# Lingeng56/conformer-pytorch-lightning

Measured on AMD Instinct MI355X. Metric: encoder frames/sec (80-d fbank, T=1000), whole job, higher is better.
Workload: dtype bf16

## Files before the change

conformer-pytorch-lightning_amd/cfm/__init__.py:

```python
import ctypes
import os
import threading

import torch

_HERE = os.path.dirname(os.path.abspath(__file__))
LIB_PATH = os.path.join(os.path.dirname(_HERE), "libconformer_gfx950.so")

F32, BF16, F16 = 0, 1, 2
ACT_NONE, ACT_SILU, ACT_RELU, ACT_GLU, ACT_DSILU, ACT_DRELU = 0, 1, 2, 3, 4, 5
TILE_AUTO_TRAIN = -1

_DT = {torch.float32: F32, torch.bfloat16: BF16, torch.float16: F16}
_TORCH_DT = {F32: torch.float32, BF16: torch.bfloat16, F16: torch.float16}

c_p = ctypes.c_void_p
c_i64 = ctypes.c_int64
c_i32 = ctypes.c_int32
c_f = ctypes.c_float


class GemmDesc(ctypes.Structure):
    _fields_ = [("A", c_p), ("W", c_p), ("W_lo", c_p), ("bias", c_p), ("residual", c_p), ("row_mask", c_p), ("C", c_p),
                ("lda", c_i64), ("ldc", c_i64), ("ldr", c_i64),
# ... 244 lines not shown
        L.cfm_dwconv_bn_train_bwd_acc.argtypes = [c_p, c_i32, c_p, c_p, c_p, c_i32, c_p, c_p, c_i32, c_p, c_p, c_p, c_p, c_p, c_p, c_i32, c_i32, c_i32, c_i32, c_i32, c_p]
        L.cfm_layernorm_bwd_fused.argtypes = [ctypes.POINTER(LnBwdDesc), c_p]
        L.cfm_conv12_relu.argtypes = [c_p, c_p, c_p, c_p, c_p, c_p, c_i32, c_i32, c_i32, c_i32, c_i32, c_p, c_p, c_p]
        L.cfm_valid_mask.argtypes = [c_p, c_i32, c_p, c_i32, c_i32, c_i32, c_i32, c_p]
        L.cfm_chunk_mask.argtypes = [c_p, c_i32, c_i32, c_i32, c_p]
        L.cfm_attn_mask.argtypes = [c_p, c_p, c_p, c_i32, c_i32, c_p]
        L.cfm_cast.argtypes = [c_p, c_i32, c_p, c_i32, c_i64, c_p]
        L.cfm_add_rows.argtypes = [c_p, c_p, c_i64, c_i32, c_i32, c_p]
        L.cfm_encoder_layer_forward.argtypes = [ctypes.POINTER(LayerWeights), ctypes.POINTER(LayerScratch),
                                                ctypes.POINTER(LayerIO), c_p, c_p, c_i32, c_p, c_p, c_p]
        L.cfm_encoder_layer_route.argtypes = [ctypes.POINTER(LayerWeights), ctypes.POINTER(LayerScratch), ctypes.POINTER(LayerIO), c_p, c_p]
        L.cfm_encoder_layer_route.restype = c_i32
        L.cfm_ffsplit_max_rows.restype = c_i32
        L.cfm_ctc_nll.argtypes = [c_p, c_i64, c_i32, c_i32, c_i32, c_p, c_p, c_i32, c_p, c_p, c_p, c_p]
        L.cfm_joint_act.argtypes = [c_p, c_i64, c_p, c_i64, c_p, c_i32, c_i32, c_i32, c_i32, c_i32, c_p]
        L.cfm_joint_act_bwd.argtypes = [c_p, c_i64, c_p, c_i64, c_p, c_p, c_p, c_p, c_i32, c_i32, c_i32, c_i32, c_p]
        L.cfm_joint_act_bwd_ws.argtypes = [c_i32, c_i32, c_i32, c_i32]
        L.cfm_rnnt_nll.argtypes = [ctypes.POINTER(RnntDesc), c_p]
        L.cfm_rnnt_grad.argtypes = [ctypes.POINTER(RnntDesc), c_p]
        L.cfm_rnnt_packed_nll.argtypes = [ctypes.POINTER(RnntPackedDesc), c_p]
        L.cfm_rnnt_packed_grad.argtypes = [ctypes.POINTER(RnntPackedDesc), c_p]
        L.cfm_joint_act_packed.argtypes = [c_p, c_i64, c_p, c_i64, c_p, c_i32, ctypes.POINTER(Lattice), c_i32, c_p]
        L.cfm_joint_act_packed_bwd.argtypes = [c_p, c_i64, c_p, c_i64, c_p, c_p, c_p, c_p, ctypes.POINTER(Lattice), c_i32, c_p]
        c_f = ctypes.c_float
        L.cfm_gemm_tn.argtypes = [ctypes.POINTER(GemmTnDesc), c_p]
        L.cfm_gemm_tn_group.argtypes = [ctypes.POINTER(GemmTnDesc), c_i32, c_p]
        L.cfm_attention_bwd.argtypes = [ctypes.POINTER(AttnBwdDesc), c_p]
        L.cfm_layernorm_bwd_ws.argtypes = [c_i64, c_i32]
        L.cfm_layernorm_bwd.argtypes = [c_p, c_p, c_i32, c_p, c_p, c_p, c_p, c_p, c_p, c_p, c_f, c_i64, c_i32, c_p]
        L.cfm_glu_bwd.argtypes = [c_p, c_i32, c_p, c_i32, c_p, c_i32, c_i64, c_i32, c_p]
        L.cfm_dwconv_bn_ws.argtypes = [c_i32, c_i32, c_i32]
        L.cfm_dwconv_bn_train.argtypes = [c_p, c_i32, c_p, c_p, c_p, c_p, c_p, c_p, c_f, c_f, c_p, c_p, c_p, c_i32, c_p, c_i32, c_i32, c_i32, c_i32, c_p]
        L.cfm_dwconv_bn_train_bwd.argtypes = [c_p, c_i32, c_p, c_p, c_p, c_i32, c_p, c_p, c_i32, c_p, c_p, c_p, c_p, c_p, c_p, c_i32, c_i32, c_i32, c_i32, c_p]
        L.cfm_col2im_relu_bwd.argtypes = [c_p, c_i32, c_p, c_i32, c_p, c_i32, c_i32, c_i32, c_i32, c_i32, c_p]
        L.cfm_conv1_wgrad_ws.argtypes = [c_i32, c_i32, c_i32]
        L.cfm_conv1_wgrad.argtypes = [c_p, c_i32, c_p, c_p, c_p, c_p, c_p, c_p, c_i32, c_i32, c_i32, c_i32, c_p]
        L.cfm_ctc_nll_train_groups.argtypes = [ctypes.POINTER(CtcGroup), c_i32, c_i32, c_p]
        L.cfm_ctc_grad.argtypes = [c_p, c_i64, c_i32, c_i32, c_i32, c_p, c_p, c_i32, c_p, c_p, c_p, c_p, c_p, c_p, c_f, c_p, c_p, c_p]
        L.cfm_adam_step.argtypes = [c_p, c_p, c_p, c_p, c_i64, c_f, c_f, c_f, c_f, c_f, c_i64, c_p, c_p]
        L.cfm_sumsq.argtypes = [c_p, c_i64, c_p, c_i32, c_p, c_p]
        L.cfm_adam_clip_step.argtypes = [c_p, c_p, c_p, c_p, c_i64, c_f, c_f, c_f, c_f, c_f, c_i64, c_p, c_f, c_f, c_i32, c_p, c_p]
        L.cfm_dropout_rows.argtypes = [c_p, c_i32, c_p, c_i32, c_p, c_f, c_f, ctypes.c_uint32, c_f, ctypes.c_uint32, c_i64, c_i32, c_p]
        L.cfm_dropout_mask.argtypes = [c_p, c_i64, c_f, ctypes.c_uint32, c_p]
        L.cfm_encoder_train_forward.argtypes = [c_i32, ctypes.POINTER(LayerTrainWeights), ctypes.POINTER(LayerTrainIO), ctypes.POINTER(LayerTrainSaved),
                                                ctypes.POINTER(LayerTrainScratch), ctypes.POINTER(c_p), c_p]
        L.cfm_encoder_train_backward.argtypes = [c_i32, ctypes.POINTER(LayerTrainWeights), ctypes.POINTER(LayerTrainIO), ctypes.POINTER(LayerTrainSaved),
                                                 ctypes.POINTER(LayerTrainScratch), ctypes.POINTER(LayerTrainGrads), ctypes.POINTER(c_p), c_p, c_p, c_p,
                                                 LAYER_DONE_FN, c_p, ctypes.POINTER(c_p), c_p]
        L.cfm_stream_prep.argtypes = [c_p, c_i32, c_i32, c_i32, c_i32, c_p, c_i32, c_i32, c_p, c_p, c_p, c_p]
        L.cfm_kv_ring_write.argtypes = [c_p, c_p, c_i32, c_i64, c_i64, c_i64, c_i64, c_p, c_p, c_i32, c_i32, c_i32, c_i32, c_i32, c_p]
        L.cfm_stream_advance.argtypes = [c_p, c_p, c_i32, c_i32, c_p]
        L.cfm_dwconv_causal_bn_silu.argtypes = [c_p, c_i32, c_p, c_p, c_p, c_p, c_p, c_p, c_i32, c_i32, c_i32, c_i32, c_i32, c_p]
        L.cfm_conv_cache_update.argtypes = [c_p, c_i32, c_p, c_i32, c_i32, c_i32, c_i32, c_p]
        for name in ("cfm_layernorm_bwd_ws", "cfm_dwconv_bn_ws", "cfm_conv1_wgrad_ws", "cfm_joint_act_bwd_ws"):
            getattr(L, name).restype = c_i64
        L.cfm_prof_enable.argtypes = [c_i32]
        L.cfm_prof_enable.restype = None
        L.cfm_prof_reset.restype = None
        L.cfm_prof_collect.restype = ctypes.c_int
        L.cfm_prof_entry.argtypes = [c_i32, ctypes.c_char_p, c_i32, ctypes.POINTER(c_i64), ctypes.POINTER(ctypes.c_double),
                                     ctypes.POINTER(ctypes.c_double), ctypes.POINTER(ctypes.c_double)]
        for name in ("cfm_gemm", "cfm_ffn_fused", "cfm_rowchain", "cfm_rowchain_supported", "cfm_attention", "cfm_layernorm", "cfm_kv_cache_pack", "cfm_dwconv_bn_silu", "cfm_conv1_relu", "cfm_conv1_relu_mma", "cfm_conv12_relu", "cfm_conv12_supported",
                     "cfm_valid_mask", "cfm_chunk_mask", "cfm_attn_mask", "cfm_cast", "cfm_add_rows",
                     "cfm_encoder_layer_forward", "cfm_ctc_nll", "cfm_joint_act", "cfm_joint_act_bwd", "cfm_rnnt_nll", "cfm_rnnt_grad", "cfm_prof_entry", "cfm_gemm_tn", "cfm_gemm_tn_group", "cfm_attention_bwd",
                     "cfm_layernorm_bwd", "cfm_glu_bwd", "cfm_dwconv_bn_train", "cfm_dwconv_bn_train_bwd", "cfm_col2im_relu_bwd", "cfm_conv1_wgrad",
                     "cfm_ctc_nll_train_groups", "cfm_ctc_grad", "cfm_adam_step", "cfm_adam_clip_step", "cfm_sumsq", "cfm_dropout_rows", "cfm_dropout_mask", "cfm_pack_matrices", "cfm_pack_vectors", "cfm_greedy_step", "cfm_greedy_chunk_begin", "cfm_greedy_chunk_step", "cfm_fbank", "cfm_fbank_stream", "cfm_ffn_split", "cfm_ffn_split_supported", "cfm_layernorm_bwd_fused", "cfm_dwconv_bn_train_bwd_acc",
                     "cfm_encoder_train_forward", "cfm_encoder_train_backward", "cfm_stream_prep", "cfm_kv_ring_write", "cfm_stream_advance", "cfm_dwconv_causal_bn_silu", "cfm_conv_cache_update"):
            getattr(L, name).restype = ctypes.c_int
        _lib = L
    return _lib


def check(rc, what):
    if rc != 0:
        raise RuntimeError("%s failed (status %d): %s" % (what, rc, lib().cfm_last_error().decode(errors="replace")))


def dt_code(t):
    try:
        return _DT[t.dtype if isinstance(t, torch.Tensor) else t]
    except KeyError:
        raise TypeError("cfm: unsupported dtype %s (float32, bfloat16, float16 only)" % (t.dtype if isinstance(t, torch.Tensor) else t))


def torch_dtype(code):
    return _TORCH_DT[code]


def require_hip(*tensors):
    for t in tensors:
        if t is None:
            continue
        if not t.is_cuda:
            raise RuntimeError("cfm: tensor on %s -- this framework runs on MI355X (HIP) only; there is no CPU path" % t.device)


def ptr(t):
    return None if t is None else t.data_ptr()


def stream():
    return torch.cuda.current_stream().cuda_stream


class Precision:

# ... 50 lines not shown
```

conformer-pytorch-lightning_amd/cfm/ops.py:

```python
import ctypes

import torch

import cfm as _c

__all__ = ["fbank", "fbank_stream", "stream_prep", "stream_advance", "dwconv_causal_bn_silu", "conv_cache_update", "dropout_rows", "dropout_mask", "set_deterministic", "gemm_tn", "gemm_tn_group", "layernorm_bwd", "glu_bwd", "dwconv_bn_train", "dwconv_bn_train_bwd", "col2im_relu_bwd", "conv1_wgrad", "attention_bwd",
           "ctc_nll_train_groups", "ctc_grad", "rnnt_nll", "rnnt_grad", "joint_act_bwd", "rnnt_nll_packed", "joint_act_packed", "joint_act_packed_bwd", "ffn_split", "adam_step", "adam_clip_step", "sumsq", "scratch_stats",
           "gemm", "ffn_fused", "ffn_fused_supported", "rowchain", "rowchain_supported", "rowchain_pair_supported", "layernorm", "attention", "kv_cache_pack", "dwconv_bn_silu", "conv1_relu", "conv1_relu_mma_supported", "conv12_relu", "conv12_supported", "ctc_nll", "joint_act", "valid_mask", "chunk_mask",
           "attn_mask_combine", "cast", "add_rows", "scratch", "prof_enable", "prof_reset", "prof_table", "as_u8_mask"]


def _rows2d(t, name):
    if t.dim() != 2 or t.stride(1) != 1:
        raise ValueError("cfm.%s: expected a 2-D tensor with unit inner stride, got shape %s strides %s" % (name, tuple(t.shape), t.stride()))
    return t


def _dense(name, **tensors):
    for k, t in tensors.items():
        if t is not None and not t.is_contiguous():
            raise ValueError("cfm.%s: %s must be contiguous (the C ABI has no stride for it), got shape %s strides %s" % (name, k, tuple(t.shape), t.stride()))


def _strides_match(name, what, t, sb, st):
    if t is None:
        return
    if t.dim() not in (2, 3):
        bad = t.stride(-1) != 1
    else:
        bad = t.stride(-1) != 1 or (t.size(-2) > 1 and t.stride(-2) != st) or (t.dim() == 3 and t.size(0) > 1 and t.stride(0) != sb)
    if bad:
        raise ValueError("cfm.%s: %s has strides %s but the call passes (batch %d, time %d) with unit inner stride" % (name, what, t.stride(), sb, st))


_arena = {}
_retired = []


def scratch(tag, numel, dtype, device):
    device = torch.device(device)
    key = (tag, dtype, device, torch.cuda.current_stream(device).cuda_stream)
    buf = _arena.get(key)
    if buf is None or buf.numel() < numel:
        want = max(int(numel), 1) if buf is None else max(int(numel), buf.numel() * 3 // 2)
        if buf is not None:
            _retired.append(buf)
        buf = torch.empty(want, dtype=dtype, device=device)
        _arena[key] = buf
    return buf[:numel]


def scratch_stats():
    held = sum(b.numel() * b.element_size() for b in list(_arena.values()) + _retired)
    return len(_arena), len(_retired), held


def gemm(a, w, bias=None, w_lo=None, out=None, out_dtype=None, act=_c.ACT_NONE, residual=None, alpha=1.0, row_mask=None,
         mask_mode=0, conv=None, tile=0, n_out=None, pre_out=None, aux=None, drop=None, drop2=None):
    _c.require_hip(a, w, bias, w_lo, out, residual, row_mask)
    w = _rows2d(w, "gemm(w)")
    N, K = w.shape
    if w.stride(0) != K:
        raise ValueError("cfm.gemm: w must be dense [N,K] (cfm_gemm_desc carries no row stride for W), got shape %s strides %s" % (tuple(w.shape), w.stride()))
    d = _c.GemmDesc()
    if conv is None:
        a = _rows2d(a, "gemm(a)")
        M = a.shape[0]
        if a.shape[1] != K:
            raise ValueError("cfm.gemm: a is %s but w is %s" % (tuple(a.shape), tuple(w.shape)))
        d.lda = a.stride(0)
    else:
        C, T1, F1, T2, F2, M = conv
        if not a.is_contiguous():
            raise ValueError("cfm.gemm(conv): image must be contiguous channels-last [B,T1,F1,C]")
        d.conv_C, d.conv_T1, d.conv_F1, d.conv_T2, d.conv_F2 = C, T1, F1, T2, F2
        d.lda = 0
    cols = N // 2 if act == _c.ACT_GLU else N
    if out is None:
        odt = out_dtype if out_dtype is not None else (residual.dtype if residual is not None else torch.float32)
        out = torch.empty((M, cols), dtype=odt, device=a.device)
    else:
        out = _rows2d(out, "gemm(out)")
        if out.shape[0] != M or out.shape[1] != cols:
            raise ValueError("cfm.gemm: out is %s, expected (%d,%d)" % (tuple(out.shape), M, cols))
    if residual is not None:
        residual = _rows2d(residual, "gemm(residual)")
        if residual.dtype != torch.float32 or out.dtype != torch.float32 or tuple(residual.shape) != (M, cols):
            raise ValueError("cfm.gemm: residual accumulate needs f32 residual/out of shape (%d,%d)" % (M, cols))
        d.ldr = residual.stride(0)
    if bias is not None and (bias.dtype != torch.float32 or bias.numel() != N or not bias.is_contiguous()):
        raise ValueError("cfm.gemm: bias must be contiguous f32 [N]")
    if row_mask is not None and (row_mask.dtype != torch.uint8 or row_mask.numel() != M or not row_mask.is_contiguous()):
        raise ValueError("cfm.gemm: row_mask must be contiguous uint8 [M]")
    if w_lo is not None and (w_lo.shape != w.shape or w_lo.dtype != w.dtype or not w_lo.is_contiguous()):
        raise ValueError("cfm.gemm: w_lo must match w")
    if pre_out is not None:
        _c.require_hip(pre_out)
        pre_out = _rows2d(pre_out, "gemm(pre_out)")
        if tuple(pre_out.shape) != (M, N):
            raise ValueError("cfm.gemm: pre_out is %s, expected (%d,%d)" % (tuple(pre_out.shape), M, N))
        d.C_pre, d.ld_pre, d.pre_dtype = _c.ptr(pre_out), pre_out.stride(0), _c.dt_code(pre_out)
    if aux is not None:
        _c.require_hip(aux)
        aux = _rows2d(aux, "gemm(aux)")
        if tuple(aux.shape) != (M, N):
            raise ValueError("cfm.gemm: aux is %s, expected (%d,%d)" % (tuple(aux.shape), M, N))
        d.aux, d.ld_aux, d.aux_dtype = _c.ptr(aux), aux.stride(0), _c.dt_code(aux)
    if drop is not None and drop[0] > 0.0:
        d.drop_p, d.drop_seed = float(drop[0]), int(drop[1]) & 0xFFFFFFFF
        if drop2 is not None and drop2[0] > 0.0:
            d.drop2_p, d.drop2_seed = float(drop2[0]), int(drop2[1]) & 0xFFFFFFFF
    d.A, d.W, d.W_lo, d.bias, d.residual, d.row_mask, d.C = _c.ptr(a), _c.ptr(w), _c.ptr(w_lo), _c.ptr(bias), _c.ptr(residual), _c.ptr(row_mask), _c.ptr(out)
    d.ldc = out.stride(0)
    d.M, d.N, d.K = M, N, K
    d.a_dtype, d.w_dtype, d.c_dtype = _c.dt_code(a), _c.dt_code(w), _c.dt_code(out)
    d.act, d.alpha, d.tile, d.mask_mode = act, alpha, tile, mask_mode
    _c.check(_c.lib().cfm_gemm(ctypes.byref(d), _c.stream()), "cfm_gemm")
    return out


def ffn_fused_supported(D, FF, prec):
    return (not prec.split) and D in (144, 256) and FF % 32 == 0 and FF <= 2048


def ffn_fused(x, w1f, w2f, b1, b2, FF, act=_c.ACT_SILU, ln=None, alpha=1.0, add_x=False, ln1=None, ln2=None, out_f32=None,
              want_f32=True, out16_dtype=None, eps=1e-5):
    _c.require_hip(x, w1f, w2f, b1, b2, out_f32)
    x = _rows2d(x, "ffn_fused(x)")
    if x.dtype != torch.float32 or not x.is_contiguous():
        raise ValueError("cfm.ffn_fused: x must be contiguous float32 [M,D]")
    M, D = x.shape
    _dense("ffn_fused", w1f=w1f, w2f=w2f, b1=b1, b2=b2, out_f32=out_f32, **{n + "_" + s: t for n, pr in (("ln", ln), ("ln1", ln1), ("ln2", ln2)) if pr is not None
                                                                            for s, t in zip("gb", pr)})
    if out_f32 is not None and (out_f32.dtype != torch.float32 or tuple(out_f32.shape) != (M, D)):
        raise ValueError("cfm.ffn_fused: out_f32 must be float32 (%d,%d)" % (M, D))
    d = _c.FfnDesc()
    d.x, d.w1f, d.w2f, d.b1, d.b2 = _c.ptr(x), _c.ptr(w1f), _c.ptr(w2f), _c.ptr(b1), _c.ptr(b2)
    for name, pair in (("ln", ln), ("ln1", ln1), ("ln2", ln2)):
        if pair is not None:
            setattr(d, name + "_g", _c.ptr(pair[0]))
            setattr(d, name + "_b", _c.ptr(pair[1]))
    if want_f32 and out_f32 is None:
        out_f32 = torch.empty((M, D), dtype=torch.float32, device=x.device)
    out16 = torch.empty((M, D), dtype=out16_dtype, device=x.device) if out16_dtype is not None else None
    d.out_f32, d.out16 = _c.ptr(out_f32), _c.ptr(out16)
    d.M, d.D, d.FF = M, D, FF
    d.w_dtype = _c.dt_code(w1f)
    d.out16_dtype = _c.dt_code(out16) if out16 is not None else 0
    d.act, d.add_x, d.alpha, d.eps = act, 1 if add_x else 0, alpha, eps
    _c.check(_c.lib().cfm_ffn_fused(ctypes.byref(d), _c.stream()), "cfm_ffn_fused")
    return out_f32, out16


def rowchain_supported(D, FF, prec):
    return (not prec.split) and bool(_c.lib().cfm_rowchain_supported(D, FF))


def rowchain_pair_supported(D, FF, prec):
    return (not prec.split) and bool(_c.lib().cfm_rowchain_pair_supported(D, FF))


def ffn_split(x, w_code, mode, psum=None, psum_b2=None, psum_alpha=1.0, ln1=None, ln2=None, rows_out=None, rows2_out=None, ln=None, w1=None, b1=None,
              n1=0, act=_c.ACT_NONE, w2=None, psum_out=None, out16=None, eps=1e-5, ring=None):
    _c.require_hip(x, psum, psum_b2, rows_out, rows2_out, w1, b1, w2, psum_out, out16)
    x = _rows2d(x, "ffn_split(x)")
    M, D = x.shape
    if x.dtype != torch.float32 or not x.is_contiguous():
        raise ValueError("cfm.ffn_split: x must be contiguous float32 rows")
    _dense("ffn_split", psum_b2=psum_b2, rows_out=rows_out, rows2_out=rows2_out, w1=w1, b1=b1, w2=w2, psum_out=psum_out,
           ring_kv=ring[0] if ring is not None else None, ring_offsets=ring[1] if ring is not None else None, **{n + "_" + sfx: t for n, pr in (("ln", ln), ("ln1", ln1), ("ln2", ln2)) if pr is not None for sfx, t in zip("gb", pr)})
# ... 848 lines not shown
```

conformer-pytorch-lightning_amd/cfm/packing.py:

```python
import torch

import cfm as _c


_EPOCH = [0]


def bump_epoch():
    _EPOCH[0] += 1


def _key(tensors, prec):
    return (prec.name, _EPOCH[0]) + tuple((t.data_ptr(), t._version, str(t.device), t.dtype) for t in tensors if t is not None)


class Packed:

    def __init__(self, **kw):
        self.__dict__.update(kw)


class PackCache:
    def __init__(self):
        self._key = None
        self._val = None

    def __reduce__(self):
        return (PackCache, ())

    def get(self, tensors, prec, build):
        k = _key(tensors, prec)
        if k != self._key:
            with torch.no_grad():
                self._val = build()
            self._key = k
        return self._val


MODULE_CACHES = ("_fused", "_grad_layout", "_stack_w", "_stack_g", "_pack_stack_train")


def state_without_caches(state):
    out = {k: v for k, v in state.items() if k not in MODULE_CACHES}
    if "_fused" in state:
        out["_fused"] = None
    return out


def f32(t):
    return t.detach().to(torch.float32).contiguous()


def matrix(w, prec):
    w32 = w.detach().to(torch.float32)
    if prec.split:
        hi = w32.to(torch.bfloat16)
        lo = (w32 - hi.to(torch.float32)).to(torch.bfloat16)
        return hi.contiguous(), lo.contiguous()
    return w32.to(prec.w_dtype).contiguous(), None


def conv_module_vectors(mod):
    D = mod.pointwise_conv2.weight.shape[0]
    dev = mod.pointwise_conv2.weight.device
    opt = lambda t, n, fill: t.detach() if t is not None else torch.full((n,), fill, device=dev)
    return opt(mod.pointwise_conv1.bias, 2 * D, 0.0), opt(mod.depthwise_conv.bias, D, 0.0), opt(mod.norm.weight, D, 1.0), opt(mod.norm.bias, D, 0.0)


def glu_interleave_index(D, device):
    idx = torch.arange(2 * D, device=device)
    return ((idx % 32) // 16) * D + (idx // 32) * 16 + (idx % 16)


def pack_ffn_fragments(w1, w2, dtype):
    FF, D = w1.shape
    ks1 = (D + 31) // 32
    w1p = torch.zeros((FF, ks1 * 32), dtype=torch.float32, device=w1.device)
    w1p[:, :D] = w1.detach().float()
    w1f = w1p.view(FF // 16, 16, ks1, 4, 8).permute(0, 2, 3, 1, 4).contiguous().to(dtype)
    w2f = w2.detach().float().view(D // 16, 16, FF // 32, 2, 4, 4).permute(2, 0, 4, 1, 3, 5).contiguous().to(dtype)
    return w1f.view(-1), w2f.view(-1)


def pack_frag_major(w, dtype):
    N, K = w.shape
    ks = (K + 31) // 32
    wp = torch.zeros((N, ks * 32), dtype=torch.float32, device=w.device)
    wp[:, :K] = w.detach().float()
    return wp.view(N // 16, 16, ks, 4, 8).permute(0, 2, 3, 1, 4).contiguous().to(dtype).view(-1)
# ... 397 lines not shown
```

conformer-pytorch-lightning_amd/csrc/encoder.cpp:

```cpp
#include <math.h>

#include <stdlib.h>

#include "cfm_common.h"

namespace {

const float kEps = 1e-5f;

inline const void* eoff(const void* p, int64_t elems, int dt) { return (const char*)p + elems * cfm_elt_size(dt); }

struct Ctx {
    const cfm_layer_weights* w; const cfm_layer_scratch* s; const cfm_layer_io* io; const float* x_in; float* x_out; cfm_stream_t st;
    int M, D, FF, H, dk, adt, w_dt, Tc, Tk, P;
    bool split, has_pos, ring;
};

int& cin_merge_flag() {
    static int flag = getenv("CFM_CIN_MERGE") == nullptr || atoi(getenv("CFM_CIN_MERGE")) != 0;
    return flag;
}

int ffsplit_max_rows() {
    static const int rows = getenv("CFM_FFSPLIT_MAX_ROWS") ? atoi(getenv("CFM_FFSPLIT_MAX_ROWS")) : CFM_FFSPLIT_MAX_ROWS;
    return rows;
}

bool taps15(const Ctx& c) { return c.io->ktaps == 15 && !c.io->causal_conv; }

#define CFM_TRY(expr) do { int rc__ = (expr); if (rc__ != CFM_OK) return rc__; } while (0)

int select_route(Ctx& c) {
    const cfm_layer_weights* w = c.w; const cfm_layer_scratch* s = c.s; const cfm_layer_io* io = c.io;
    CFM_CHECK_ARG(w && s && io && c.x_in && c.x_out, "cfm_encoder_layer_forward: null pointer");
    CFM_CHECK_ARG(io->B > 0 && io->T > 0 && io->D > 0 && io->H > 0 && io->D % io->H == 0 && io->FF > 0,
                  "cfm_encoder_layer_forward: bad dims B=%d T=%d D=%d H=%d FF=%d", io->B, io->T, io->D, io->H, io->FF);
    CFM_CHECK_ARG(io->D % 16 == 0, "cfm_encoder_layer_forward: D must be a multiple of 16 (GLU interleave)");
    CFM_CHECK_ARG(c.x_in != c.x_out, "cfm_encoder_layer_forward: x_in and x_out must differ (inputs are not mutated)");
    c.M = io->B * io->T; c.D = io->D; c.FF = io->FF; c.H = io->H; c.dk = c.D / c.H; c.adt = io->act_dtype; c.w_dt = io->w_dtype;
    c.split = io->act_dtype == CFM_F32;
    c.has_pos = io->pos_rows > 0 && w->pos_w;
    c.ring = io->kv_ring != nullptr;
    CFM_CHECK_ARG(!c.ring || (io->stream_offset && io->ring_T >= io->T && !io->attn_cache && !io->new_cache),
                  "encoder layer: the K/V ring needs stream_offset and ring_T >= T, and excludes attn_cache / new_cache");
    c.Tc = io->attn_cache ? io->cache_T : 0;
    c.Tk = c.ring ? io->ring_T : c.Tc + io->T;
    c.P = 0;
    if (c.has_pos) {
        CFM_CHECK_ARG((io->pos_embed || io->pos_proj) && (io->pos_shared || io->pos_rows % io->B == 0),
                      "encoder layer: pos_embed rows (%d) must be a multiple of B (%d)", io->pos_rows, io->B);
        c.P = io->pos_shared ? io->pos_rows : io->pos_rows / io->B;
        CFM_CHECK_ARG(!io->pos_shared || c.P == c.Tk, "encoder layer: shared positions need one row per key (%d rows, Tk=%d)", io->pos_rows, c.Tk);
        CFM_CHECK_ARG(c.P == 1 || c.P == c.Tk, "encoder layer: pos_embed gives %d rows per item, need 1 or Tk=%d (attention.py:78-88)", c.P, c.Tk);
    }
    CFM_CHECK_ARG(c.Tc == 0 || io->new_cache, "encoder layer: a KV cache input needs new_cache storage");
// ... 247 lines not shown
    return cfm_rowchain(&fi, c.st);
}

int run_ffsplit(const Ctx& c) {
    const cfm_layer_weights* w = c.w; const cfm_layer_io* io = c.io;
    const bool ring_written = c.ring && c.dk % 4 == 0;
    CFM_TRY(split_ffn(c, true, c.x_in));
    cfm_ffn_split_desc q = split_reduce(c, 1, c.x_in, w->ffm_b2);
    q.ln_g = w->ln_mha_g; q.ln_b = w->ln_mha_b; q.w1 = w->qkv_wf; q.b1 = w->qkv_b; q.N1 = 3 * c.D; q.act = CFM_ACT_NONE; q.out16 = c.s->qkv; q.ldo = 3 * c.D;
    if (ring_written) { q.kv_ring = io->kv_ring; q.ring_offsets = io->stream_offset; q.ring_T = io->ring_T; q.ring_H = c.H; q.ring_Tq = io->T; }
    CFM_TRY(cfm_ffn_split(&q, c.st));
    CFM_TRY(attention(c, ring_written));
    CFM_TRY(conv_in_chain(c));
    CFM_TRY(conv_out(c, taps15(c) && cfm_rowchain_dw_supported(c.D), c.x_out, 0));
    CFM_TRY(split_ffn(c, false, c.x_out));
    cfm_ffn_split_desc r = split_reduce(c, 0, c.x_out, w->ff_b2);
    r.ln1_g = w->ln_final_g; r.ln1_b = w->ln_final_b;
    if (io->after_out) { r.ln2_g = io->after_g; r.ln2_b = io->after_b; r.rows2_out = io->after_out; }
    return cfm_ffn_split(&r, c.st);
}

int run_pair(const Ctx& c) {
    const cfm_layer_weights* w = c.w; const cfm_layer_scratch* s = c.s;
    float* const park = s->psum + (int64_t)2 * c.M * c.D;
    cfm_rowchain_desc m = ffn_chain(c, true, c.x_in);
    m.psum_out = s->psum;
    CFM_TRY(cfm_rowchain(&m, c.st));
    cfm_rowchain_desc q = chain(c, 1.0f);
    q.x = c.x_in; q.psum_in = s->psum; q.psum_b2 = w->ffm_b2; q.psum_alpha = 0.5f; q.out_f32 = c.x_out; q.ln_g = w->ln_mha_g; q.ln_b = w->ln_mha_b; q.tail_pair = 1;
    qkv_tail(q, c, w);
    CFM_TRY(cfm_rowchain(&q, c.st));
    CFM_TRY(attention(c));
    CFM_TRY(conv_in_chain(c, park));
    CFM_TRY(conv_out(c, taps15(c), park, 1));
    cfm_rowchain_desc fa = ffn_chain(c, false, c.x_out);
    fa.psum_out = s->psum;
    CFM_TRY(cfm_rowchain(&fa, c.st));
    cfm_rowchain_desc fr = chain(c, 1.0f);
    fr.x = c.x_out; fr.psum_in = s->psum; fr.psum_b2 = w->ff_b2; fr.psum_alpha = 0.5f; fr.ln_g = w->ln_final_g; fr.ln_b = w->ln_final_b; fr.out2_f32 = c.x_out;
    CFM_TRY(cfm_rowchain(&fr, c.st));
    return after_norm(c);
}

}

extern "C" int32_t cfm_set_cin_merge(int32_t on) {
    const int prev = cin_merge_flag();
    cin_merge_flag() = on != 0;
    return prev;
}

extern "C" int32_t cfm_ffsplit_max_rows(void) { return ffsplit_max_rows(); }

extern "C" int32_t cfm_encoder_layer_route(const cfm_layer_weights* w, const cfm_layer_scratch* s, const cfm_layer_io* io, const float* x_in, const float* x_out) {
    Ctx c = {w, s, io, x_in, const_cast<float*>(x_out), nullptr};
    return select_route(c);
}

extern "C" int cfm_encoder_layer_forward(const cfm_layer_weights* w, const cfm_layer_scratch* s, const cfm_layer_io* io,
                                         const float* x_in, float* x_out, int xn_ready, const float* next_g,
                                         const float* next_b, cfm_stream_t stream) {
    Ctx c = {w, s, io, x_in, x_out, stream};
    const int route = select_route(c);
    switch (route) {
        case CFM_ROUTE_GENERAL: return run_general(c, xn_ready, next_g, next_b);
        case CFM_ROUTE_FUSED_FFN: return run_fused_ffn(c);
        case CFM_ROUTE_CHAIN: return run_chain(c);
        case CFM_ROUTE_CHAIN_NEXT: return run_chain_next(c);
        case CFM_ROUTE_CHAIN_NEXT_CIN: return run_chain_next_cin(c);
        case CFM_ROUTE_FFSPLIT: return run_ffsplit(c);
        case CFM_ROUTE_PAIR: return run_pair(c);
        default: return route;
    }
}
```

conformer-pytorch-lightning_amd/encoder.py:

```python
import torch
import torch.nn as nn

import cfm
from attention import PositionalEncoding, RelativePositionalEncoding
from convolution import ConvolutionSubSampling
from encoder_layer import ConformerEncoderLayer
from utils import make_attn_mask, make_pad_mask

_NO_MASK = torch.ones((0, 0, 0))


class ConformerEncoder(nn.Module):

    def __init__(self, input_dim, kernel_size, encoder_dim, dropout, attention_dropout, pos_enc_dropout, hidden_dim,
                 num_heads, encoder_num_layers, cmvn=None, max_len=5000, use_relative=False, use_dynamic_chunk_size=False,
                 use_dynamic_left_chunk=False, static_chunk_size=-1):
        super().__init__()
        pe_cls = RelativePositionalEncoding if use_relative else PositionalEncoding
        self.position_encoding = pe_cls(encoder_dim, pos_enc_dropout, max_len)
        self.embed = ConvolutionSubSampling(input_dim=input_dim, output_dim=encoder_dim, pos_enc=self.position_encoding)
        self.encoders = nn.ModuleList([
            ConformerEncoderLayer(encoder_dim, kernel_size, dropout, attention_dropout, hidden_dim, num_heads, use_relative)
            for _ in range(encoder_num_layers)])
        self.encoder_dim = encoder_dim
# ... 6 lines not shown
    def _run_blocks(self, x, attn_mask, pos_embed, pad_mask, caches, keep_from, pos_shared=False, proj=None, ring=None, conv=None, streaming=False):
        n = len(self.encoders)
        if proj is None:
            proj = self._project_positions(pos_embed, x)
        bufs = [torch.empty_like(x), torch.empty_like(x)]
        new_caches = [] if caches is not None else None
        cur, ready = x, False
        prec = cfm.resolve_precision(self)
        fuse_after = (cfm.rowchain_supported(self.encoder_dim, self.encoders[0].hidden_dim, prec) and
                      self.after_norm.weight.dtype == torch.float32 and self.after_norm.eps == 1e-5)
        y_after = torch.empty_like(x) if fuse_after else None
        import encoder_layer as _el
        e0 = self.encoders[0]
        chain = (_el.CHAIN_BLOCKS and fuse_after and caches is None and conv is None and self.encoder_dim == 256 and
                 e0.hidden_dim == 2048 and e0.kernel_size == 15 and not getattr(e0.conv_module, "causal", False) and
                 all(b.chain_ready(prec) for b in self.encoders) and
                 not (streaming and _el.SPLIT_FFN_FEW_ROWS and _el.split_rows(x.size(0) * x.size(1), self.encoder_dim, e0.hidden_dim)))
        for i, block in enumerate(self.encoders):
            nxt = self.encoders[i + 1].norm_ff_macaron if i + 1 < n else None
            cache_i = None
            if caches is not None and caches.dim() == 5 and caches.size(0) > 0:
                cache_i = caches[i]
            elif caches is not None and caches.dim() == 4 and caches.size(0) > 0:
                cache_i = caches[i:i + 1]
            pp = None if proj is None else (proj[:, i * self.encoder_dim:], proj.stride(0))
            out, nc = block.fused_forward(cur, attn_mask, pos_embed, pad_mask, cache_i, xn_ready=ready, next_norm=nxt,
                                          out=bufs[i & 1], want_cache=caches is not None, pos_proj=pp, pos_shared=pos_shared,
                                          ring=None if ring is None else (ring[0][i], ring[1]), conv_cache=None if conv is None else conv[i],
                                          chain_next=(self.encoders[i + 1], bufs[(i + 1) & 1]) if chain and i + 1 < n else None,
                                          macaron_done=chain and i > 0, split_ffn=streaming,
                                          after=(self.after_norm.weight.detach(), self.after_norm.bias.detach(), y_after)
                                          if fuse_after and i + 1 == n else None)
            if new_caches is not None:
                new_caches.append(nc[:, :, keep_from:, :])
            cur, ready = out, nxt is not None
        if fuse_after:
            return y_after, new_caches
        y, _ = cfm.layernorm(cur.view(-1, cur.size(-1)), self.after_norm.weight.detach(), self.after_norm.bias.detach(),
                             eps=self.after_norm.eps)
        return y.view_as(cur), new_caches

    def _cmvn_args(self, inputs):
        m = self.global_cmvn
        if m is None:
            return inputs, None
        mean, istd = getattr(m, "mean", None), getattr(m, "istd", None)
        ok = (isinstance(mean, torch.Tensor) and isinstance(istd, torch.Tensor) and mean.dtype == torch.float32 and istd.dtype == torch.float32 and
              mean.dim() == 1 and mean.shape == istd.shape and mean.numel() == inputs.size(-1) and mean.device == inputs.device and
              inputs.dtype == torch.float32)
        if not ok:
            return m(inputs), None
        return inputs, (mean.contiguous(), istd.contiguous() if getattr(m, "norm_var", True) else None)

    def _project_positions(self, pos_embed, x):
        if not isinstance(self.position_encoding, RelativePositionalEncoding) or pos_embed is None:
            return None
        from cfm import packing
        prec = cfm.resolve_precision(self)
        ws = [blk.self_attn.linear_pos.weight for blk in self.encoders]
        if not hasattr(self, "_pos_pack"):
            self._pos_pack = packing.PackCache()
        pk = self._pos_pack.get(ws, prec, lambda: packing.Packed(w=packing.matrix(torch.cat([w.detach() for w in ws], 0), prec)))
        pe = pos_embed.reshape(-1, self.encoder_dim)
        pe = (pe if pe.dtype == torch.float32 else pe.float()).contiguous()
        return cfm.gemm(pe, pk.w[0], w_lo=pk.w[1], out_dtype=prec.act_dtype)

    def __getstate__(self):
        from cfm import packing
        return packing.state_without_caches(super().__getstate__())

    def set_precision(self, name):
        prec = None if name is None else (name if isinstance(name, cfm.Precision) else cfm.Precision(name))
        for m in self.modules():
            m.precision = prec
        return self

    def forward(self, inputs, input_lengths, decoding_chunk_size=0, num_decoding_chunk_size=-1):
        if self.training:
            return self.forward_window([(inputs, input_lengths)], decoding_chunk_size, num_decoding_chunk_size)[0]
        inputs, cmvn = self._cmvn_args(inputs)
        cfm.require_hip(inputs, input_lengths)
        frames = inputs.size(1)
        x = self.embed.embed_frames(inputs, cmvn)
        x, pos_embed = self.position_encoding(x, 0)
        pad_mask = cfm.valid_mask(input_lengths, x.size(1), first=6, stride=4).unsqueeze(1)
        attn_mask = make_attn_mask(x, pad_mask, self.use_dynamic_chunk_size, self.use_dynamic_left_chunk,
                                   decoding_chunk_size, self.static_chunk_size, num_decoding_chunk_size)
        y, _ = self._run_blocks(x, attn_mask, pos_embed, pad_mask, None, 0, streaming=bool(getattr(self, "split_small_batches", False)))
        return y.to(inputs.dtype), pad_mask

    def forward_window(self, batches, decoding_chunk_size=0, num_decoding_chunk_size=-1, return_rows=False):
        if not self.training:
            raise RuntimeError("ConformerEncoder.forward_window is the train-mode pass over an accumulation window; in eval mode call forward per batch")
        from cfm import autograd as ag
        from encoder_layer import _mask_args
        layers = list(self.encoders)
        flat = all(l.__dict__.get("_flat_leaf") is not None for l in layers)
        ag.check_params(layers, flat)
        if not ag.stack_supported(layers, len(batches)):
            outs = []
            for inputs, lengths in batches:
                inputs, cmvn = self._cmvn_args(inputs)
                cfm.require_hip(inputs, lengths)
                x, pos_embed = self.position_encoding(self.embed.embed_frames(inputs, cmvn), 0)
                pad_mask = cfm.valid_mask(lengths, x.size(1), first=6, stride=4).unsqueeze(1)
                attn_mask = make_attn_mask(x, pad_mask, self.use_dynamic_chunk_size, self.use_dynamic_left_chunk, decoding_chunk_size,
                                           self.static_chunk_size, num_decoding_chunk_size)
                for block in layers:
                    x, attn_mask, _, _ = block(x, attn_mask, pos_embed, pad_mask)
                y = ag.LayerNormFn.apply(x, self.after_norm.weight, self.after_norm.bias, self.after_norm.eps)
                outs.append((y.to(inputs.dtype), pad_mask))
            if return_rows:
                return torch.cat([y.float().reshape(-1, y.size(-1)) for y, _ in outs], 0), outs
            return outs
        prec = cfm.resolve_precision(self)
        rows, groups, keeps, shapes, pads = [], [], [], [], []
        for gi, (inputs, lengths) in enumerate(batches):
            inputs, cmvn = self._cmvn_args(inputs)
            cfm.require_hip(inputs, lengths)
            x, pos_embed = self.position_encoding(self.embed.embed_frames(inputs, cmvn), 0)
            B, T, D = x.shape
            pad_mask = cfm.valid_mask(lengths, T, first=6, stride=4).unsqueeze(1)
            attn_mask = make_attn_mask(x, pad_mask, self.use_dynamic_chunk_size, self.use_dynamic_left_chunk, decoding_chunk_size,
                                       self.static_chunk_size, num_decoding_chunk_size)
            m8, m_str = _mask_args(attn_mask, B, T, T)
            cfm.require_hip(m8)
            rows.append(x.reshape(B * T, D))
            groups.append((B, T, m8, m_str))
            keeps.append(cfm.as_u8_mask(pad_mask).reshape(-1))
            shapes.append((B, T, inputs.dtype))
            pads.append(pad_mask)
        x_rows = rows[0] if len(rows) == 1 else torch.cat(rows, 0)
        x_rows = (x_rows if x_rows.dtype == torch.float32 else x_rows.float()).contiguous()
        keep = keeps[0] if len(keeps) == 1 else torch.cat(keeps, 0)
        params = tuple(l.__dict__["_flat_leaf"] for l in layers) if flat else tuple(p for l in layers for p in l.parameters())
        y = ag.EncoderStackFn.apply(x_rows, self, layers, prec, groups, keep, flat, *params)
        y = ag.LayerNormFn.apply(y, self.after_norm.weight, self.after_norm.bias, self.after_norm.eps)
        outs, r0 = [], 0
        for (B, T, dt), pad_mask in zip(shapes, pads):
            outs.append((y[r0:r0 + B * T].view(B, T, -1).to(dt), pad_mask))
            r0 += B * T
# ... 256 lines not shown
```

include/cfm.h:

```cpp
#ifndef CFM_H_
#define CFM_H_

#include <stddef.h>
#include <stdint.h>

#ifdef __cplusplus
extern "C" {
#endif

#define CFM_VERSION 306

typedef void* cfm_stream_t;

typedef enum { CFM_F32 = 0, CFM_BF16 = 1, CFM_F16 = 2 } cfm_dtype;

typedef enum {
    CFM_OK = 0,
    CFM_ERR_ARG = -1,
    CFM_ERR_LAUNCH = -2,
    CFM_ERR_UNSUPPORTED = -3
} cfm_status;

typedef enum {
    CFM_ACT_NONE = 0, CFM_ACT_SILU = 1, CFM_ACT_RELU = 2, CFM_ACT_GLU = 3,
// ... 201 lines not shown
} cfm_layer_weights;

typedef struct {
    void *xn, *hid, *qkv, *pos, *ctx, *glu, *dw;
    float* psum;
    int32_t psum_splits;
} cfm_layer_scratch;
#define CFM_PAIR_MAX_ROWS 4096
#define CFM_FFSPLIT_MAX_ROWS 1536

typedef struct {
    int32_t B, T, D, H, FF, ktaps;
    int32_t act_dtype;
    int32_t w_dtype;
    const uint8_t* attn_mask;
    int64_t am_sb, am_sq;
    const uint8_t* pad_valid;
    const float* pos_embed;
    int32_t pos_rows;
    const void* pos_proj;
    int64_t pos_proj_ld;
    const float* attn_cache;
    int32_t cache_T;
    float* new_cache;
    const float *after_g, *after_b;
    float* after_out;
    float* kv_ring;
    const int32_t* stream_offset;
    int32_t ring_T;
    int32_t causal_conv;
    float* conv_cache;
    int32_t pos_shared;
    const cfm_layer_weights* next_w;
    float* next_x_out;
    int32_t macaron_done;
} cfm_layer_io;

typedef enum {
    CFM_ROUTE_GENERAL = 0,
    CFM_ROUTE_FUSED_FFN = 1,
    CFM_ROUTE_CHAIN = 2,
    CFM_ROUTE_CHAIN_NEXT = 3,
    CFM_ROUTE_CHAIN_NEXT_CIN = 4,
    CFM_ROUTE_FFSPLIT = 5,
    CFM_ROUTE_PAIR = 6
} cfm_route;

int cfm_encoder_layer_forward(const cfm_layer_weights* w, const cfm_layer_scratch* s, const cfm_layer_io* io,
                              const float* x_in, float* x_out, int xn_ready, const float* next_g,
                              const float* next_b, cfm_stream_t stream);
int32_t cfm_encoder_layer_route(const cfm_layer_weights* w, const cfm_layer_scratch* s, const cfm_layer_io* io, const float* x_in, const float* x_out);
int32_t cfm_ffsplit_max_rows(void);

int cfm_ctc_nll(const float* logits, int64_t ld, int32_t B, int32_t T, int32_t V, const int32_t* enc_lens,
                const int32_t* labels, int32_t Umax, const int32_t* label_lens, float* work, float* nll, cfm_stream_t stream);

int cfm_joint_act(const float* enc, int64_t ld_e, const float* pred, int64_t ld_p, void* out, int32_t out_dtype, int32_t B,
                  int32_t T, int32_t U, int32_t J, cfm_stream_t stream);

typedef struct {
    const void* logits;
    int64_t ld;
    int32_t logits_dtype;
    int32_t B, T, U1, V, blank;
    const int32_t* targets;
    const int32_t* logit_lens;
    const int32_t* target_lens;
    float *lse, *lp_blank, *lp_label, *alpha, *beta, *shift;
    float *nll, *nll_shifted, *ll_alpha;
    void* grad;
    int64_t ld_grad;
    int32_t grad_dtype, grad_cols;
    float gscale;
    int32_t gscale_stride;
    const float* gscale_dev;
    float clamp;
} cfm_rnnt_desc;
int cfm_rnnt_nll(const cfm_rnnt_desc* d, cfm_stream_t stream);
int cfm_rnnt_grad(const cfm_rnnt_desc* d, cfm_stream_t stream);

int64_t cfm_joint_act_bwd_ws(int32_t B, int32_t T, int32_t U, int32_t J);
int cfm_joint_act_bwd(const float* enc, int64_t ld_e, const float* pred, int64_t ld_p, const float* dact, float* d_enc, float* d_pred,
                      float* work, int32_t B, int32_t T, int32_t U, int32_t J, cfm_stream_t stream);

typedef struct {
    int32_t B, T_max, U1_max;
    int64_t M;
    const int64_t* off;
    const int32_t* T;
    const int32_t* U;
    const int64_t* enc_row0;
    const int64_t* pred_row0;
    int64_t n_enc, n_pred;
    const int64_t* blk_off;
} cfm_lattice;

int cfm_joint_act_packed(const float* enc, int64_t ld_e, const float* pred, int64_t ld_p, void* out, int32_t out_dtype, const cfm_lattice* lat,
                         int32_t J, cfm_stream_t stream);
int cfm_joint_act_packed_bwd(const float* enc, int64_t ld_e, const float* pred, int64_t ld_p, const float* dact, float* d_enc, float* d_pred,
                             float* work, const cfm_lattice* lat, int32_t J, cfm_stream_t stream);

typedef struct {
    cfm_lattice lat;
    const void* logits;
    int64_t ld;
    int32_t logits_dtype, V, blank, ld_targets;
// ... 267 lines not shown
```

Before: 27.38 million.

## Cache relative-position projection across eval forwards keyed on weights and table version

Adds a native cache for the stacked linear_pos projection of the positional-encoding table. In eval mode, when the position embedding is a contiguous fp32 view of the stored table, a repeat call with identical weights, table version, pointers and shapes skips the GEMM and reuses the prior output buffer. A hit from another stream is gated on a HIP event. The projection is computed once and passed to the block runner. This removes a per-forward GEMM that depends only on parameters, at the cost of host-side key checks, a mutex and stream-capture special cases.

```diff
diff --git a/conformer-pytorch-lightning_amd/cfm/__init__.py b/conformer-pytorch-lightning_amd/cfm/__init__.py
--- a/conformer-pytorch-lightning_amd/cfm/__init__.py
+++ b/conformer-pytorch-lightning_amd/cfm/__init__.py
@@ -320,6 +320,16 @@
         L.cfm_stream_advance.argtypes = [c_p, c_p, c_i32, c_i32, c_p]
         L.cfm_dwconv_causal_bn_silu.argtypes = [c_p, c_i32, c_p, c_p, c_p, c_p, c_p, c_p, c_i32, c_i32, c_i32, c_i32, c_i32, c_p]
         L.cfm_conv_cache_update.argtypes = [c_p, c_i32, c_p, c_i32, c_i32, c_i32, c_i32, c_p]
+        L.cfm_pos_cache_create.argtypes = []
+        L.cfm_pos_cache_create.restype = c_p
+        L.cfm_pos_cache_destroy.argtypes = [c_p]
+        L.cfm_pos_cache_destroy.restype = None
+        L.cfm_pos_cache_invalidate.argtypes = [c_p]
+        L.cfm_pos_cache_invalidate.restype = None
+        L.cfm_pos_cache_project.argtypes = [c_p, ctypes.POINTER(GemmDesc), ctypes.c_uint64, c_p, c_i64, ctypes.c_uint64, c_p, ctypes.POINTER(c_i32)]
+        L.cfm_pos_cache_project.restype = ctypes.c_int
+        L.cfm_set_pos_cache.argtypes = [c_i32]
+        L.cfm_set_pos_cache.restype = c_i32
         for name in ("cfm_layernorm_bwd_ws", "cfm_dwconv_bn_ws", "cfm_conv1_wgrad_ws", "cfm_joint_act_bwd_ws"):
             getattr(L, name).restype = c_i64
         L.cfm_prof_enable.argtypes = [c_i32]
diff --git a/conformer-pytorch-lightning_amd/cfm/ops.py b/conformer-pytorch-lightning_amd/cfm/ops.py
--- a/conformer-pytorch-lightning_amd/cfm/ops.py
+++ b/conformer-pytorch-lightning_amd/cfm/ops.py
@@ -56,7 +56,7 @@
 
 
 def gemm(a, w, bias=None, w_lo=None, out=None, out_dtype=None, act=_c.ACT_NONE, residual=None, alpha=1.0, row_mask=None,
-         mask_mode=0, conv=None, tile=0, n_out=None, pre_out=None, aux=None, drop=None, drop2=None):
+         mask_mode=0, conv=None, tile=0, n_out=None, pre_out=None, aux=None, drop=None, drop2=None, enqueue=None):
     _c.require_hip(a, w, bias, w_lo, out, residual, row_mask)
     w = _rows2d(w, "gemm(w)")
     N, K = w.shape
@@ -115,7 +115,10 @@
     d.M, d.N, d.K = M, N, K
     d.a_dtype, d.w_dtype, d.c_dtype = _c.dt_code(a), _c.dt_code(w), _c.dt_code(out)
     d.act, d.alpha, d.tile, d.mask_mode = act, alpha, tile, mask_mode
-    _c.check(_c.lib().cfm_gemm(ctypes.byref(d), _c.stream()), "cfm_gemm")
+    if enqueue is not None:
+        enqueue(d)
+    else:
+        _c.check(_c.lib().cfm_gemm(ctypes.byref(d), _c.stream()), "cfm_gemm")
     return out
 
 
diff --git a/conformer-pytorch-lightning_amd/cfm/packing.py b/conformer-pytorch-lightning_amd/cfm/packing.py
--- a/conformer-pytorch-lightning_amd/cfm/packing.py
+++ b/conformer-pytorch-lightning_amd/cfm/packing.py
@@ -35,6 +35,47 @@
                 self._val = build()
             self._key = k
         return self._val
+
+
+_POS_VERSION = [0]
+
+
+class PosProjCache:
+
+    def __init__(self):
+        self._h = _c.lib().cfm_pos_cache_create()
+        if not self._h:
+            raise MemoryError("cfm_pos_cache_create")
+        _POS_VERSION[0] += 1
+        self.version = _POS_VERSION[0]
+        self.bufs = {}
+        self.computed = 0
+
+    def __reduce__(self):
+        return (PosProjCache, ())
+
+    def __del__(self):
+        h, self._h = getattr(self, "_h", None), None
+        if h:
+            try:
+                _c.lib().cfm_pos_cache_destroy(h)
+            except Exception:
+                pass
+
+    def project(self, rows, table, w, w_lo, out_dtype):
+        import ctypes
+        key = (rows.size(0), w.size(0), out_dtype, str(rows.device))
+        out = self.bufs.get(key)
+        if out is None:
+            out = self.bufs[key] = torch.empty((rows.size(0), w.size(0)), dtype=out_dtype, device=rows.device)
+        ran = ctypes.c_int32(0)
+
+        def enqueue(d):
+            _c.check(_c.lib().cfm_pos_cache_project(self._h, ctypes.byref(d), self.version, table.data_ptr(), table.size(0), table._version,
+                                                    _c.stream(), ctypes.byref(ran)), "cfm_pos_cache_project")
+        _c.gemm(rows, w, w_lo=w_lo, out=out, enqueue=enqueue)
+        self.computed += ran.value
+        return out
 
 
 MODULE_CACHES = ("_fused", "_grad_layout", "_stack_w", "_stack_g", "_pack_stack_train")
diff --git a/conformer-pytorch-lightning_amd/csrc/encoder.cpp b/conformer-pytorch-lightning_amd/csrc/encoder.cpp
--- a/conformer-pytorch-lightning_amd/csrc/encoder.cpp
+++ b/conformer-pytorch-lightning_amd/csrc/encoder.cpp
@@ -1,6 +1,9 @@
 #include <math.h>
 
 #include <stdlib.h>
+
+#include <mutex>
+#include <new>
 
 #include "cfm_common.h"
 
@@ -354,6 +357,112 @@
 
 extern "C" int32_t cfm_ffsplit_max_rows(void) { return ffsplit_max_rows(); }
 
+namespace {
+
+struct PosKey {
+    uint64_t pack_version, table_version;
+    const void *table, *A, *W, *W_lo, *C;
+    int64_t table_rows, lda, ldc;
+    int M, N, K, a_dtype, w_dtype, c_dtype;
+    bool operator==(const PosKey& o) const {
+        return pack_version == o.pack_version && table_version == o.table_version && table == o.table && A == o.A && W == o.W && W_lo == o.W_lo && C == o.C &&
+               table_rows == o.table_rows && lda == o.lda && ldc == o.ldc && M == o.M && N == o.N && K == o.K && a_dtype == o.a_dtype &&
+               w_dtype == o.w_dtype && c_dtype == o.c_dtype;
+    }
+};
+
+struct PosEntry {
+    bool valid = false;
+    PosKey key;
+    hipStream_t stream = nullptr;
+    hipEvent_t done = nullptr;
+};
+
+int& pos_cache_flag() {
+    static int flag = getenv("CFM_POS_CACHE") == nullptr || atoi(getenv("CFM_POS_CACHE")) != 0;
+    return flag;
+}
+
+}
+
+struct cfm_pos_cache {
+    static constexpr int kEntries = 8;
+    std::mutex mu;
+    PosEntry e[kEntries];
+    int next = 0;
+};
+
+extern "C" cfm_pos_cache* cfm_pos_cache_create(void) { return new (std::nothrow) cfm_pos_cache(); }
+
+extern "C" void cfm_pos_cache_destroy(cfm_pos_cache* c) {
+    if (!c) return;
+    for (PosEntry& e : c->e)
+        if (e.done) (void)hipEventDestroy(e.done);
+    delete c;
+}
+
+extern "C" void cfm_pos_cache_invalidate(cfm_pos_cache* c) {
+    if (!c) return;
+    std::lock_guard<std::mutex> lock(c->mu);
+    for (PosEntry& e : c->e) e.valid = false;
+}
+
+extern "C" int32_t cfm_set_pos_cache(int32_t on) {
+    const int prev = pos_cache_flag();
+    pos_cache_flag() = on != 0;
+    return prev;
+}
+
+extern "C" int cfm_pos_cache_project(cfm_pos_cache* c, const cfm_gemm_desc* d, uint64_t pack_version, const void* table, int64_t table_rows,
+                                     uint64_t table_version, cfm_stream_t stream, int32_t* computed) {
+    CFM_CHECK_ARG(c && d && d->A && d->W && d->C, "cfm_pos_cache_project: null pointer");
+    CFM_CHECK_ARG(!d->bias && !d->residual && !d->row_mask && d->act == CFM_ACT_NONE && !d->C_pre && !d->aux && d->drop_p == 0.f && d->conv_C == 0,
+                  "cfm_pos_cache_project: a plain product only (linear_pos has no bias; attention.py:78)");
+    if (computed) *computed = 1;
+    hipStream_t s = (hipStream_t)stream;
+    if (!pos_cache_flag()) return cfm_gemm(d, stream);
+    const PosKey key = {pack_version, table_version, table, d->A, d->W, d->W_lo, d->C, table_rows, d->lda, d->ldc, d->M, d->N, d->K, d->a_dtype, d->w_dtype, d->c_dtype};
+    std::lock_guard<std::mutex> lock(c->mu);
+    PosEntry* hit = nullptr;
+    for (PosEntry& e : c->e)
+        if (e.valid && e.key == key) hit = &e;
+    if (hit) {
+        bool usable = hit->stream == s;
+        if (!usable) {
+            usable = hipEventQuery(hit->done) == hipSuccess;
+            (void)hipGetLastError();
+        }
+        if (usable) {
+            if (computed) *computed = 0;
+            return CFM_OK;
+        }
+        return cfm_gemm(d, stream);
+    }
+    hipStreamCaptureStatus cap = hipStreamCaptureStatusNone;
+    if (hipStreamIsCapturing(s, &cap) != hipSuccess) {
+        (void)hipGetLastError();
+        cap = hipStreamCaptureStatusActive;
+    }
+    CFM_TRY(cfm_gemm(d, stream));
+    if (cap != hipStreamCaptureStatusNone) return CFM_OK;
+    for (PosEntry& e : c->e)
+        if (e.valid && e.key.C == key.C) e.valid = false;
+    PosEntry& e = c->e[c->next];
+    c->next = (c->next + 1) % cfm_pos_cache::kEntries;
+    e.valid = false;
+    if (!e.done && hipEventCreateWithFlags(&e.done, hipEventDisableTiming) != hipSuccess) {
+        (void)hipGetLastError();
+        e.done = nullptr;
+        return CFM_OK;
+    }
+    if (hipEventRecord(e.done, s) != hipSuccess) {
+        (void)hipGetLastError();
+        return CFM_OK;
+    }
+    e.key = key; e.stream = s; e.valid = true;
+    return CFM_OK;
+}
+
 extern "C" int32_t cfm_encoder_layer_route(const cfm_layer_weights* w, const cfm_layer_scratch* s, const cfm_layer_io* io, const float* x_in, const float* x_out) {
     Ctx c = {w, s, io, x_in, const_cast<float*>(x_out), nullptr};
     return select_route(c);
diff --git a/conformer-pytorch-lightning_amd/encoder.py b/conformer-pytorch-lightning_amd/encoder.py
--- a/conformer-pytorch-lightning_amd/encoder.py
+++ b/conformer-pytorch-lightning_amd/encoder.py
@@ -82,7 +82,7 @@
             return m(inputs), None
         return inputs, (mean.contiguous(), istd.contiguous() if getattr(m, "norm_var", True) else None)
 
-    def _project_positions(self, pos_embed, x):
+    def _project_positions(self, pos_embed, x, table=None):
         if not isinstance(self.position_encoding, RelativePositionalEncoding) or pos_embed is None:
             return None
         from cfm import packing
@@ -90,8 +90,13 @@
         ws = [blk.self_attn.linear_pos.weight for blk in self.encoders]
         if not hasattr(self, "_pos_pack"):
             self._pos_pack = packing.PackCache()
-        pk = self._pos_pack.get(ws, prec, lambda: packing.Packed(w=packing.matrix(torch.cat([w.detach() for w in ws], 0), prec)))
+        pk = self._pos_pack.get(ws, prec, lambda: packing.Packed(w=packing.matrix(torch.cat([w.detach() for w in ws], 0), prec), proj=None))
         pe = pos_embed.reshape(-1, self.encoder_dim)
+        if (table is not None and not self.training and pe.dtype == torch.float32 and pe.is_contiguous() and
+                pe.untyped_storage().data_ptr() == table.untyped_storage().data_ptr()):
+            if pk.proj is None:
+                pk.proj = packing.PosProjCache()
+            return pk.proj.project(pe, table, pk.w[0], pk.w[1], prec.act_dtype)
         pe = (pe if pe.dtype == torch.float32 else pe.float()).contiguous()
         return cfm.gemm(pe, pk.w[0], w_lo=pk.w[1], out_dtype=prec.act_dtype)
 
@@ -116,7 +121,8 @@
         pad_mask = cfm.valid_mask(input_lengths, x.size(1), first=6, stride=4).unsqueeze(1)
         attn_mask = make_attn_mask(x, pad_mask, self.use_dynamic_chunk_size, self.use_dynamic_left_chunk,
                                    decoding_chunk_size, self.static_chunk_size, num_decoding_chunk_size)
-        y, _ = self._run_blocks(x, attn_mask, pos_embed, pad_mask, None, 0, streaming=bool(getattr(self, "split_small_batches", False)))
+        proj = self._project_positions(pos_embed, x, table=self.position_encoding.pe)
+        y, _ = self._run_blocks(x, attn_mask, pos_embed, pad_mask, None, 0, proj=proj, streaming=bool(getattr(self, "split_small_batches", False)))
         return y.to(inputs.dtype), pad_mask
 
     def forward_window(self, batches, decoding_chunk_size=0, num_decoding_chunk_size=-1, return_rows=False):
diff --git a/include/cfm.h b/include/cfm.h
--- a/include/cfm.h
+++ b/include/cfm.h
@@ -277,6 +277,14 @@
 int32_t cfm_encoder_layer_route(const cfm_layer_weights* w, const cfm_layer_scratch* s, const cfm_layer_io* io, const float* x_in, const float* x_out);
 int32_t cfm_ffsplit_max_rows(void);
 
+typedef struct cfm_pos_cache cfm_pos_cache;
+cfm_pos_cache* cfm_pos_cache_create(void);
+void cfm_pos_cache_destroy(cfm_pos_cache* c);
+void cfm_pos_cache_invalidate(cfm_pos_cache* c);
+int cfm_pos_cache_project(cfm_pos_cache* c, const cfm_gemm_desc* d, uint64_t pack_version, const void* table, int64_t table_rows,
+                          uint64_t table_version, cfm_stream_t stream, int32_t* computed);
+int32_t cfm_set_pos_cache(int32_t on);
+
 int cfm_ctc_nll(const float* logits, int64_t ld, int32_t B, int32_t T, int32_t V, const int32_t* enc_lens,
                 const int32_t* labels, int32_t Umax, const int32_t* label_lens, float* work, float* nll, cfm_stream_t stream);
 
```

Result: slower. 27.10 million (-1.0%).
